# aim-uofa/GenPercept

Measured on AMD Instinct MI355X. Metric: images/sec at 768x768 bf16 (depth), higher is better.
Workload: dtype bf16

## Files before the change

genpercept_amd/csrc/attention.hip:

```cpp
#include <cstdlib>

#include "common.h"
#include "kernels.h"

GP_DEV int attn_off128(int row, int slot) { return row * 128 + ((slot ^ ((row >> 1) & 7)) << 4); }

#ifndef GP_FLASH_DEFER
#define GP_FLASH_DEFER 0.f
#endif
template <int NKB, int NST>
__global__ __launch_bounds__(256, 2) void flash_attn64_kernel(const h16_t* __restrict__ Q, const h16_t* __restrict__ K,
                                                            const h16_t* __restrict__ Vt, h16_t* __restrict__ O, int T, int heads, int ldq,
                                                            int ldk, int Tpad, int ldo) {
    constexpr int KEYS = 32 * NKB, KBYTES = KEYS * 128, NH = NKB / 2;
    constexpr int STAGE = 2 * KBYTES;
    extern __shared__ __attribute__((aligned(16))) char smem[];
    const int tid = threadIdx.x, lane = tid & 63;
    const int wave = __builtin_amdgcn_readfirstlane(tid >> 6);
    const int nqb = (T + 127) >> 7;
    const int sid = xcd_remap(blockIdx.x, gridDim.x);
    const int qb = sid % nqb, bh = sid / nqb;
    const int h = bh % heads, b = bh / heads;
    const int q0 = qb * 128 + wave * 32;
    const int l31 = lane & 31, hh = lane >> 5;
// ... 449 lines not shown
                fr[ks % F5_RD] = lds_frag(sb + (ka0 ^ ((ks & 7) << 5)), (ks >> 3) * 256);
                if ((ks & 3) == 3) ql[(ks >> 2) & 1] = lds_frag(q_lds, (ks >> 2) * 1024);
            };
#pragma unroll
            for (int ks = 0; ks < F5_RD; ++ks) rd(ks);
#pragma unroll
            for (int ks = 0; ks < 32; ++ks) {
                const h16x8_t qv = (ks & 3) != 3 ? qf[3 * (ks >> 2) + ((ks & 3) != 3 ? (ks & 3) : 0)] : ql[(ks >> 2) & 1];
                if (ks & 1) s1 = mfma_32x32x16(fr[ks % F5_RD], qv, ks == 1 ? zero16 : s1);
                else s0 = mfma_32x32x16(fr[ks % F5_RD], qv, ks == 0 ? zero16 : s0);
                if (ks + F5_RD < 32) rd(ks + F5_RD);
                if (do_stage && (ks & 1)) stage_piece(slot_next, kt + 1, ks >> 1);
            }
            f32x16_t s_acc;
#pragma unroll
            for (int r = 0; r < 16; ++r) s_acc[r] = s0[r] + s1[r];
            if (MASK) {
                const int kbase = kt * 32 + 8 * hh;
#pragma unroll
                for (int r = 0; r < 16; ++r)
                    if (kbase + (r & 7) + 16 * (r >> 3) >= T) s_acc[r] = -1e30f;
            }
            float mx = s_acc[0];
#pragma unroll
            for (int r = 1; r < 16; ++r) mx = fmaxf(mx, s_acc[r]);
            mx = fmaxf(mx, other_half(mx));
            const bool moved = __builtin_amdgcn_ballot_w64((mx - m_run) * sc > 8.f) != 0ull;
            if (moved) {
                const float m_new = fmaxf(m_run, mx);
                alpha = __builtin_amdgcn_exp2f((m_run - m_new) * sc);
                m_run = m_new;
                l_run *= alpha;
            }
            const float nm = -m_run * sc;
            float rs = 0.f;
#pragma unroll
            for (int r = 0; r < 16; ++r) {
                s_acc[r] = __builtin_amdgcn_exp2f(__builtin_fmaf(s_acc[r], sc, nm));
                rs += s_acc[r];
            }
            l_run += rs;
#pragma unroll
            for (int j = 0; j < 2; ++j) {
                union { h16x8_t v; unsigned u[4]; } t;
#pragma unroll
                for (int e = 0; e < 4; ++e) t.u[e] = pack_h16x2_ns(s_acc[8 * j + 2 * e], s_acc[8 * j + 2 * e + 1]);
                pf[j] = t.v;
            }
            return moved;
        };
        auto pv_phase = [&](unsigned sb) __attribute__((always_inline)) {
            h16x8_t fr[F5_RD];
            auto rd = [&](int st) __attribute__((always_inline)) { fr[st % F5_RD] = lds_frag(sb + va[st >> 4], (st & 15) * 2048); };
#pragma unroll
            for (int st = 0; st < F5_RD; ++st) rd(st);
#pragma unroll
            for (int st = 0; st < 32; ++st) {
                o_acc[st & 15] = mfma_32x32x16(fr[st % F5_RD], pf[st >> 4], o_acc[st & 15]);
                if (st + F5_RD < 32) rd(st + F5_RD);
            }
        };

        if (t0 < t1) stage(0, t0);
        __builtin_amdgcn_s_waitcnt(0x0070);
        int kt = t0;
        for (;;) {
            bool pending = false;
            unsigned sb = 0;
            for (; kt < t1; ++kt) {
                const int rel = (kt - t0) & 1;
                sb = smem_base + rel * F5_KBYTES;
                wait_vm<0>();
                __builtin_amdgcn_s_barrier();
                const bool nx = kt + 1 < t1;
                const bool moved = (kt * 32 + 32 > T) ? s_phase(sb, kt, nx, rel ^ 1, IC<1>{}) : s_phase(sb, kt, nx, rel ^ 1, IC<0>{});
                if (moved) { pending = true; break; }
                pv_phase(sb);
            }
            if (!pending) break;
#pragma unroll
            for (int d = 0; d < 16; ++d) {
#pragma unroll
                for (int r = 0; r < 16; ++r) o_acc[d][r] *= alpha;
                __builtin_amdgcn_sched_barrier(0);
            }
            pv_phase(sb);
            ++kt;
            __builtin_amdgcn_s_waitcnt(0x0070);
        }
        l_run += other_half(l_run);
        const int q = q0 + l31;
        if (whole) {
            const float inv = 1.f / l_run;
            if (q < T) {
                h16_t* ob = O + ((long long)b * T + q) * ldo;
#pragma unroll
                for (int d = 0; d < 16; ++d)
#pragma unroll
                    for (int g = 0; g < 4; ++g) {
                        const uint2 pk = pack_h16x4(o_acc[d][4 * g] * inv, o_acc[d][4 * g + 1] * inv, o_acc[d][4 * g + 2] * inv, o_acc[d][4 * g + 3] * inv);
                        *(uint2*)(ob + d * 32 + 8 * g + 4 * hh) = pk;
                    }
            }
        } else {
            const long long slot = (long long)(sid / S) * S + part;
            float* po = part_o + (slot * 128 + wave * 32 + l31) * 512;
#pragma unroll
            for (int d = 0; d < 16; ++d)
#pragma unroll
                for (int g = 0; g < 4; ++g)
                    *(float4*)(po + d * 32 + 8 * g + 4 * hh) = float4{o_acc[d][4 * g], o_acc[d][4 * g + 1], o_acc[d][4 * g + 2], o_acc[d][4 * g + 3]};
            if (hh == 0) {
                float* pm = part_ml + (slot * 128 + wave * 32 + l31) * 2;
                pm[0] = m_run;
                pm[1] = l_run;
            }
        }
    }
}

__global__ __launch_bounds__(256) void flash512_combine_kernel(const float* __restrict__ part_o, const float* __restrict__ part_ml,
                                                                h16_t* __restrict__ O, int T, int nqb, int first_blk, int Li, int S, int ldo,
                                                                float scale) {
    const int lb = blockIdx.x >> 2, qq = (blockIdx.x & 3) * 32 + (threadIdx.x >> 3);
    const int b = Li ? lb / Li : (first_blk + lb) / nqb;
    const int q = (Li ? nqb - Li + (lb - b * Li) : first_blk + lb - b * nqb) * 128 + qq;
    if (q >= T) return;
    const float sc = scale * 1.44269504088896340736f;
    float m = -1e30f;
    for (int p = 0; p < S; ++p) m = fmaxf(m, part_ml[(((long long)lb * S + p) * 128 + qq) * 2]);
    float l = 0.f;
    float acc[64];
#pragma unroll
    for (int i = 0; i < 64; ++i) acc[i] = 0.f;
    const int c0 = (threadIdx.x & 7) * 4;
    for (int p = 0; p < S; ++p) {
        const long long row = ((long long)lb * S + p) * 128 + qq;
        const float w = __builtin_amdgcn_exp2f((part_ml[row * 2] - m) * sc);
        l += w * part_ml[row * 2 + 1];
        const float* po = part_o + row * 512 + c0;
#pragma unroll
        for (int i = 0; i < 16; ++i) {
            const float4 v = *(const float4*)(po + 32 * i);
            acc[4 * i] += w * v.x; acc[4 * i + 1] += w * v.y; acc[4 * i + 2] += w * v.z; acc[4 * i + 3] += w * v.w;
        }
    }
    const float inv = 1.f / l;
    h16_t* ob = O + ((long long)b * T + q) * ldo + c0;
#pragma unroll
    for (int i = 0; i < 16; ++i)
        *(uint2*)(ob + 32 * i) = pack_h16x4(acc[4 * i] * inv, acc[4 * i + 1] * inv, acc[4 * i + 2] * inv, acc[4 * i + 3] * inv);
}

bool flash_attn512_supported(int C) { return C == 512 && !gp_sw().no_flash512; }
static int flash512_grid(int nblocks, int ncu, int T) {
    if (nblocks >= ncu) return ncu;
    const int nt = (T + 31) / 32;
    int parts = ncu / nblocks;
    if (parts > nt / 8) parts = nt / 8;
    return parts >= 2 ? parts * nblocks : nblocks;
}
long long flash_attn512_workspace_floats(int B, int T, int ncu) {
    const int nblocks = B * ((T + 127) / 128), G = flash512_grid(nblocks, ncu, T);
    const int L = nblocks % G;
    return L ? (long long)(G / L) * L * 128 * (512 + 2) : 0;
}
void launch_flash_attn512(const h16_t* q, const h16_t* k, const h16_t* vt, h16_t* out, float* ws, int B, int T, int ldq,
                          int ldk, int Tpad, int ldo, float scale, int ncu, hipStream_t s) {
    static unsigned long long attr_mask = 0;
    gp_once_per_device(&attr_mask, [&] { (void)hipFuncSetAttribute((const void*)flash_attn512_kernel, hipFuncAttributeMaxDynamicSharedMemorySize, F5_LDS); });
    const int nqb = (T + 127) / 128, nblocks = B * nqb, G = flash512_grid(nblocks, ncu, T);
    const int rounds = nblocks / G, L = nblocks - rounds * G, S = L ? G / L : 0;
    float* part_o = ws;
    float* part_ml = ws ? ws + (long long)S * L * 128 * 512 : nullptr;
    const int dbg = gp_sw().f5_dbg;
    hipLaunchKernelGGL(flash_attn512_kernel, dim3(G), dim3(256), F5_LDS, s, q, k, vt, out, part_o, part_ml, B, T, ldq, ldk, Tpad,
                       ldo, scale, dbg);
    if (L) hipLaunchKernelGGL(flash512_combine_kernel, dim3(L * 4), dim3(256), 0, s, part_o, part_ml, out, T, nqb, rounds * G, (L % B == 0) ? L / B : 0,
                              S, ldo, scale);
}

__global__ __launch_bounds__(256) void cross_attn_small_kernel(const h16_t* __restrict__ q, const float* __restrict__ kc,
                                                                const float* __restrict__ vc, h16_t* __restrict__ out, long long nrh,
                                                                int C, int heads, int L) {
    const long long idx = (long long)blockIdx.x * 256 + threadIdx.x;
    if (idx >= nrh) return;
    const long long row = idx / heads;
    const int h = (int)(idx - row * heads);
    float qv[64];
    const h16_t* qp = q + row * C + h * 64;
#pragma unroll
    for (int i = 0; i < 8; ++i) {
        const uint4 raw = *(const uint4*)(qp + i * 8);
        const unsigned w[4] = {raw.x, raw.y, raw.z, raw.w};
#pragma unroll
        for (int k = 0; k < 4; ++k) { qv[i * 8 + 2 * k] = h16_lo(w[k]); qv[i * 8 + 2 * k + 1] = h16_hi(w[k]); }
    }
    float o[64];
#pragma unroll
    for (int d = 0; d < 64; ++d) o[d] = 0.f;
    float m = -1e30f, l = 0.f;
    for (int j = 0; j < L; ++j) {
        const float* kp = kc + (long long)j * C + h * 64;
        float s = 0.f;
#pragma unroll
        for (int d = 0; d < 64; ++d) s += qv[d] * kp[d];
        s *= 0.125f;
        const float mn = fmaxf(m, s);
        const float a = __expf(m - mn), pj = __expf(s - mn);
        m = mn;
        l = l * a + pj;
        const float* vp = vc + (long long)j * C + h * 64;
#pragma unroll
        for (int d = 0; d < 64; ++d) o[d] = o[d] * a + pj * vp[d];
    }
    const float inv = 1.f / l;
    h16_t* op = out + row * C + h * 64;
#pragma unroll
    for (int i = 0; i < 8; ++i) {
        uint4 r;
        r.x = pack_h16x2(o[i * 8] * inv, o[i * 8 + 1] * inv);
        r.y = pack_h16x2(o[i * 8 + 2] * inv, o[i * 8 + 3] * inv);
        r.z = pack_h16x2(o[i * 8 + 4] * inv, o[i * 8 + 5] * inv);
        r.w = pack_h16x2(o[i * 8 + 6] * inv, o[i * 8 + 7] * inv);
        *(uint4*)(op + i * 8) = r;
    }
}

void launch_cross_attn_small(const h16_t* q, const float* kc, const float* vc, h16_t* out, int rows, int C, int L, hipStream_t s) {
    const int heads = C / 64;
    const long long nrh = (long long)rows * heads;
    hipLaunchKernelGGL(cross_attn_small_kernel, dim3((unsigned)((nrh + 255) / 256)), dim3(256), 0, s, q, kc, vc, out, nrh, C, heads, L);
}

__global__ __launch_bounds__(256) void softmax_rows_kernel(const float* __restrict__ in, h16_t* __restrict__ out, int T, int ld, float scale) {
    __shared__ float red[8];
    const long long row = blockIdx.x;
    const float* x = in + row * ld;
    h16_t* y = out + row * ld;
    const int tid = threadIdx.x, lane = tid & 63, wv = tid >> 6;
    const float sc = scale * 1.44269504088896340736f;
    float mx = -1e30f;
    for (int i = tid; i < T; i += 256) mx = fmaxf(mx, x[i] * sc);
#pragma unroll
    for (int o = 32; o > 0; o >>= 1) mx = fmaxf(mx, __shfl_xor(mx, o));
    if (lane == 0) red[wv] = mx;
    __syncthreads();
    mx = fmaxf(fmaxf(red[0], red[1]), fmaxf(red[2], red[3]));
    float sum = 0.f;
    for (int i = tid; i < T; i += 256) sum += exp2f(x[i] * sc - mx);
#pragma unroll
    for (int o = 32; o > 0; o >>= 1) sum += __shfl_xor(sum, o);
    if (lane == 0) red[4 + wv] = sum;
    __syncthreads();
    const float inv = 1.f / (red[4] + red[5] + red[6] + red[7]);
    for (int i = tid; i < ld; i += 256) y[i] = i < T ? f_to_h16(exp2f(x[i] * sc - mx) * inv) : (h16_t)0;
}

GP_DEV float4 load4(const float* p, int i) { return ((const float4*)p)[i]; }
GP_DEV float4 load4(const _Float16* p, int i) {
    typedef _Float16 h4_t __attribute__((ext_vector_type(4)));
    const h4_t h = ((const h4_t*)p)[i];
    return make_float4((float)h[0], (float)h[1], (float)h[2], (float)h[3]);
}
template <int NV, typename TIN>
__global__ __launch_bounds__(256) void softmax_rows_reg_kernel(const TIN* __restrict__ in, h16_t* __restrict__ out, int T, int ld, float scale) {
    __shared__ float red[8];
    const long long row = blockIdx.x;
    const TIN* x = in + row * ld;
    uint2* y = (uint2*)(out + row * ld);
    const int tid = threadIdx.x, lane = tid & 63, wv = tid >> 6;
    const float sc = scale * 1.44269504088896340736f;
    const int nvec = ld >> 2;
    float4 v[NV];
    float mx = -1e30f;
#pragma unroll
    for (int k = 0; k < NV; ++k) {
        const int i = k * 256 + tid;
        v[k] = i < nvec ? load4(x, i) : make_float4(0.f, 0.f, 0.f, 0.f);
        const int e0 = i * 4;
        v[k].x = e0 + 0 < T ? v[k].x : -1e30f;
        v[k].y = e0 + 1 < T ? v[k].y : -1e30f;
        v[k].z = e0 + 2 < T ? v[k].z : -1e30f;
        v[k].w = e0 + 3 < T ? v[k].w : -1e30f;
        mx = fmaxf(mx, fmaxf(fmaxf(v[k].x, v[k].y), fmaxf(v[k].z, v[k].w)));
    }
#pragma unroll
    for (int o = 32; o > 0; o >>= 1) mx = fmaxf(mx, __shfl_xor(mx, o));
    if (lane == 0) red[wv] = mx;
    __syncthreads();
    mx = fmaxf(fmaxf(red[0], red[1]), fmaxf(red[2], red[3]));
    const float nm = -mx * sc;
    float sum = 0.f;
#pragma unroll
    for (int k = 0; k < NV; ++k) {
        v[k].x = __builtin_amdgcn_exp2f(__builtin_fmaf(v[k].x, sc, nm));
        v[k].y = __builtin_amdgcn_exp2f(__builtin_fmaf(v[k].y, sc, nm));
        v[k].z = __builtin_amdgcn_exp2f(__builtin_fmaf(v[k].z, sc, nm));
        v[k].w = __builtin_amdgcn_exp2f(__builtin_fmaf(v[k].w, sc, nm));
        sum += (v[k].x + v[k].y) + (v[k].z + v[k].w);
    }
#pragma unroll
    for (int o = 32; o > 0; o >>= 1) sum += __shfl_xor(sum, o);
    if (lane == 0) red[4 + wv] = sum;
    __syncthreads();
    const float inv = 1.f / (red[4] + red[5] + red[6] + red[7]);
#pragma unroll
    for (int k = 0; k < NV; ++k) {
        const int i = k * 256 + tid;
        if (i < nvec) y[i] = pack_h16x4(v[k].x * inv, v[k].y * inv, v[k].z * inv, v[k].w * inv);
    }
}

void launch_softmax_rows(const float* in, h16_t* out, int rows, int T, int ld, float scale, hipStream_t s) {
    if ((ld & 3) == 0 && scale > 0.f && ld <= 16384) {
        if (ld <= 4096) hipLaunchKernelGGL((softmax_rows_reg_kernel<4, float>), dim3(rows), dim3(256), 0, s, in, out, T, ld, scale);
        else if (ld <= 9216) hipLaunchKernelGGL((softmax_rows_reg_kernel<9, float>), dim3(rows), dim3(256), 0, s, in, out, T, ld, scale);
        else hipLaunchKernelGGL((softmax_rows_reg_kernel<16, float>), dim3(rows), dim3(256), 0, s, in, out, T, ld, scale);
        return;
    }
    hipLaunchKernelGGL(softmax_rows_kernel, dim3(rows), dim3(256), 0, s, in, out, T, ld, scale);
}

bool softmax_rows_f16_supported(int ld) { return (ld & 3) == 0 && ld <= 16384; }
void launch_softmax_rows_f16(const void* in, h16_t* out, int rows, int T, int ld, float scale, hipStream_t s) {
    const _Float16* x = (const _Float16*)in;
    if (ld <= 4096) hipLaunchKernelGGL((softmax_rows_reg_kernel<4, _Float16>), dim3(rows), dim3(256), 0, s, x, out, T, ld, scale);
    else if (ld <= 9216) hipLaunchKernelGGL((softmax_rows_reg_kernel<9, _Float16>), dim3(rows), dim3(256), 0, s, x, out, T, ld, scale);
    else hipLaunchKernelGGL((softmax_rows_reg_kernel<16, _Float16>), dim3(rows), dim3(256), 0, s, x, out, T, ld, scale);
}
// ... 3 lines not shown
```

genpercept_amd/csrc/igemm.hip:

```cpp
#include <cstdlib>
#include <cstring>

#include "common.h"
#include "epilogue.h"
#include "kernels.h"

#include <atomic>

std::mutex& gp_attr_mutex() {
    static std::mutex m;
    return m;
}

static GpSwitches g_switches = [] {
    GpSwitches s{};
    s.gn_fuse_max_slices = s.gn_fuse_below_px = s.vt_tile = s.xfold_lds = -1;
    s.qkv_fuse_max_rows = 1 << 30;
    return s;
}();
const GpSwitches& gp_sw() { return g_switches; }
void gp_switches_reload() {
    auto flag = [](const char* n) { return getenv(n) != nullptr ? 1 : 0; };
    auto num = [](const char* n, int dflt) { const char* v = getenv(n); return v ? atoi(v) : dflt; };
    GpSwitches s{};
    s.flash_ring3 = flag("GENPERCEPT_FLASH_RING3");
    s.no_flash512 = flag("GENPERCEPT_NO_FLASH512");
    s.f5_dbg = num("GENPERCEPT_F5_DBG", 0);
    s.no_conv_few = flag("GENPERCEPT_NO_CONV_FEW");
    s.no_conv_img = flag("GENPERCEPT_NO_CONV_IMG");
    s.conv_img_s = num("GENPERCEPT_CONV_IMG_S", 0);
    s.no_cross_fold = flag("GENPERCEPT_NO_CROSS_FOLD");
    s.no_gn_fusion = flag("GENPERCEPT_NO_GN_FUSION");
    s.gn_fuse_max_slices = num("GENPERCEPT_GN_FUSE_MAX_SLICES", -1);
    s.gn_fuse_below_px = num("GENPERCEPT_GN_FUSE_BELOW_PX", -1);
    s.no_stats_fusion = flag("GENPERCEPT_NO_STATS_FUSION");
    s.vt_tile = num("GENPERCEPT_VT_TILE", -1);
    s.no_gn_small = flag("GENPERCEPT_NO_GN_SMALL");
    s.fp32_scores = flag("GENPERCEPT_FP32_SCORES");
    s.no_qkv_fuse = flag("GENPERCEPT_NO_QKV_FUSE");
    s.qkv_fuse_max_rows = num("GENPERCEPT_QKV_FUSE_MAX_ROWS", 1 << 30);
    s.no_rgb_conv = flag("GENPERCEPT_NO_RGB_CONV");
    s.igemm_dbg = num("GENPERCEPT_IGEMM_DBG", 0);
    s.no_splitk = flag("GENPERCEPT_NO_SPLITK");
    s.no_halo = flag("GENPERCEPT_NO_HALO");
    s.no_pgemm = flag("GENPERCEPT_NO_PGEMM");
    s.gn_apply_old = flag("GENPERCEPT_GN_APPLY_OLD");
    s.no_up_phases = flag("GENPERCEPT_NO_UP_PHASES");
    s.gn_small_old = flag("GENPERCEPT_GN_SMALL_OLD");
    s.xfold_lds = num("GENPERCEPT_XFOLD_LDS", -1);
    s.no_fin_fuse = flag("GENPERCEPT_NO_FIN_FUSE");
    s.c_no_flash = flag("GENPERCEPT_C_NO_FLASH");
    s.pgemm_ring3 = flag("GENPERCEPT_PGEMM_RING3");
    static std::mutex mu;
    std::lock_guard<std::mutex> lk(mu);
    if (memcmp(&g_switches, &s, sizeof(s)) != 0) g_switches = s;
}

constexpr bool PRIO = true;
template <int N>
GP_DEV void wait_vm_n() { asm volatile("s_waitcnt vmcnt(%0)" ::"n"(N) : "memory"); }

template <int BM, int BN, int WM, int WN, int KS, int NSTAGE>
__global__ __launch_bounds__(64 * WM * WN) void igemm_kernel(const IGemmParams p) {
    constexpr int NW = WM * WN;
    constexpr int TM = BM / WM, TN = BN / WN;
    constexpr int FM = TM / 16, FN = TN / 16, FP = FN / 2;
    constexpr int A_IT = BM / (8 * NW), B_IT = BN / (8 * NW);
    constexpr int LPS = A_IT + B_IT;
    constexpr int A_BYTES = BM * 128, STAGE = (BM + BN) * 128;
    constexpr bool CONV = KS != 1, UPS = KS == 4;
    static_assert((NW == 4 || NW == 8) && TM % 16 == 0 && TN % 32 == 0 && BM % (8 * NW) == 0 && BN % (8 * NW) == 0, "tile shape");
    static_assert(NSTAGE >= 2 && NSTAGE <= 4, "ring depth");
    extern __shared__ __attribute__((aligned(16))) char smem[];

    const int tid = threadIdx.x, lane = tid & 63;
    const int wave = __builtin_amdgcn_readfirstlane(tid >> 6);
    const int wm = wave / WN, wn = wave % WN;
    const bool second_half = wave >= NW / 2;

    const int ncols = p.N > p.n_store ? p.N : p.n_store;
    const int tiles_n = (ncols + BN - 1) / BN, tiles_m = (p.M + BM - 1) / BM;
    const int sid = xcd_remap(blockIdx.x, tiles_m * tiles_n);
    const int m0 = (sid / tiles_n) * BM, n0 = (sid % tiles_n) * BN;
    const int z = blockIdx.y;

    const h16_t* in = p.in + (long long)z * p.in_bs;
    const h16_t* wt = p.wt + (long long)z * p.wt_bs;
    const int Cin = p.Cin;
    const int cpt = Cin >> 6;
    const int nk_all = (CONV ? 9 : 1) * cpt;
    const int zs = p.ksplit > 1 ? (int)blockIdx.z : 0;
    const int k_begin = p.ksplit > 1 ? (int)((long long)nk_all * zs / p.ksplit) : 0;
    const int nk = p.ksplit > 1 ? (int)((long long)nk_all * (zs + 1) / p.ksplit) - k_begin : nk_all;

    const int chunk_a = (lane & 7) ^ (lane >> 3);
    const int chunk_w = (lane & 7) ^ (((lane >> 4) & 1) | ((wave & 1) << 1) | (((wave >> 1) & 1) << 2));
    const h16_t* zsrc_a = p.zero + chunk_a * 8;
    const h16_t* zsrc_w = p.zero + chunk_w * 8;

    const h16_t* a_base[A_IT];
    unsigned a_mask[A_IT];
    int a_y0[UPS ? A_IT : 1], a_x0[UPS ? A_IT : 1];
    const h16_t* a_tap[UPS ? A_IT : 1];
#pragma unroll
    for (int i = 0; i < A_IT; ++i) {
        const int m = m0 + (wave + NW * i) * 8 + (lane >> 3);
        const bool ok = m < p.M;
        if (!CONV) {
            a_base[i] = in + (long long)m * p.lda + chunk_a * 8;
            a_mask[i] = ok ? 1u : 0u;
        } else {
            const int hw = p.Ho * p.Wo;
            const int b = m / hw, rem = m - b * hw;
            const int oy = rem / p.Wo, ox = rem - oy * p.Wo;
            const int y0 = oy * p.stride - p.pad_t, x0 = ox * p.stride - p.pad_l;
            const h16_t* img = in + (long long)b * p.Hi * p.Wi * Cin + chunk_a * 8;
            unsigned mk = 0;
            const int hlim = UPS ? p.Hu : p.Hi, wlim = UPS ? p.Wu : p.Wi;
#pragma unroll
            for (int t = 0; t < 9; ++t)
                if (ok && (unsigned)(y0 + t / 3) < (unsigned)hlim && (unsigned)(x0 + t % 3) < (unsigned)wlim) mk |= 1u << t;
            a_mask[i] = mk;
            if constexpr (UPS) {
                a_base[i] = img;
                a_y0[i] = y0;
                a_x0[i] = x0;
                a_tap[i] = img;
            } else {
                a_base[i] = img + ((long long)y0 * p.Wi + x0) * Cin;
            }
        }
    }
    const h16_t* w_base[B_IT];
    bool w_ok[B_IT];
#pragma unroll
    for (int i = 0; i < B_IT; ++i) {
        const int n = n0 + (wave + NW * i) * 8 + (lane >> 3);
        w_ok[i] = n < p.n_rows;
        w_base[i] = wt + (long long)n * p.ldw + chunk_w * 8;
    }
    const float ups_sy = UPS ? (float)p.Hi / (float)p.Hu : 1.f;
    const float ups_sx = UPS ? (float)p.Wi / (float)p.Wu : 1.f;

    int st_tap = CONV ? k_begin / cpt : 0, st_cc = CONV ? k_begin - st_tap * cpt : k_begin;
    int st_ky = st_tap / 3, st_kx = st_tap - 3 * st_ky;
    auto stage = [&](int buf) {
        char* sb = smem + buf * STAGE;
        if constexpr (UPS) {
          if (st_cc == 0) {
#pragma unroll
            for (int i = 0; i < A_IT; ++i) {
                const int iy = min((int)floorf((float)(a_y0[i] + st_ky) * ups_sy), p.Hi - 1);
                const int ix = min((int)floorf((float)(a_x0[i] + st_kx) * ups_sx), p.Wi - 1);
                a_tap[i] = a_base[i] + ((long long)iy * p.Wi + ix) * Cin;
            }
          }
        }
        const int koff = st_cc << 6;
        const long long aoff = CONV && !UPS ? (long long)(st_ky * p.Wi + st_kx) * Cin + koff : koff;
#pragma unroll
        for (int i = 0; i < A_IT; ++i) {
            const bool ok = (a_mask[i] >> st_tap) & 1u;
            const h16_t* ab;
            if constexpr (UPS) ab = a_tap[i]; else ab = a_base[i];
            const h16_t* src = ok ? ab + aoff : zsrc_a;
            glds16(src, sb + (wave + NW * i) * 1024);
        }
        const int woff = st_tap * Cin + koff;
#pragma unroll
        for (int i = 0; i < B_IT; ++i) {
            const h16_t* src = w_ok[i] ? w_base[i] + woff : zsrc_w;
            glds16(src, sb + A_BYTES + (wave + NW * i) * 1024);
        }
        if (++st_cc == cpt) {
            st_cc = 0;
            if (CONV) {
                ++st_tap;
                if (++st_kx == 3) { st_kx = 0; ++st_ky; }
            }
        }
// ... 245 lines not shown
```

genpercept_amd/csrc/kernels.h:

```cpp
#pragma once
#include <hip/hip_runtime.h>
#include <stdint.h>

#include <mutex>

#ifndef GP_F16
#define GP_F16 0
#endif
typedef unsigned short h16_t;

enum { GP_ACT_NONE = 0, GP_ACT_SILU = 1, GP_ACT_RELU = 2, GP_ACT_GEGLU = 3 };
enum { GP_BIAS_NONE = 0, GP_BIAS_COL = 1, GP_BIAS_ROW = 2 };

struct IGemmParams {
    const h16_t* in;
    const h16_t* wt;
    const float* bias;
    const h16_t* res;
    void* out;
    const h16_t* zero;
    const float* in_scale;
    const float* in_shift;
    int in_silu;
    float* stats_out;
    int M, N, Cin;
    int n_rows;
    int ks;
    int B, Hi, Wi, Ho, Wo;
    int stride, pad_t, pad_l;
    int ups;
    int Hu, Wu;
    int lda, ldo, ldres;
    int ldw;
    int n_store;
    int out_fp32;
    int act, bias_mode;
    int dbg;
    float* splitk_ws;
    long long splitk_ws_floats;
    int batch;
    int ksplit;
    long long split_bs;
    long long in_bs, wt_bs, out_bs, res_bs, bias_bs;
    h16_t* vt_out;
    int vt_col0, vt_T, vt_Tpad;
    const h16_t* wt_ph;
    int res_f32;
};

struct GpSwitches {
    int flash_ring3, no_flash512, f5_dbg, no_conv_few, no_conv_img, conv_img_s, no_cross_fold, no_gn_fusion, gn_fuse_max_slices,
        gn_fuse_below_px, no_stats_fusion, vt_tile, no_gn_small, fp32_scores, no_qkv_fuse, qkv_fuse_max_rows, no_rgb_conv, igemm_dbg, no_splitk,
        no_halo, no_pgemm, gn_apply_old, xfold_lds, no_fin_fuse, pgemm_ring3, gn_small_old, no_up_phases, c_no_flash;
};
const GpSwitches& gp_sw();
void gp_switches_reload();

void* gp_sat_flag_addr_igemm();
void* gp_sat_flag_addr_conv_halo();
void* gp_sat_flag_addr_pgemm();
void* gp_sat_flag_addr_conv_few();
void* gp_sat_flag_addr_norm();
void* gp_sat_flag_addr_attention();
void* gp_sat_flag_addr_elementwise();
#define GP_SAT_TUS {gp_sat_flag_addr_igemm, gp_sat_flag_addr_conv_halo, gp_sat_flag_addr_pgemm, gp_sat_flag_addr_conv_few, gp_sat_flag_addr_norm, gp_sat_flag_addr_attention, gp_sat_flag_addr_elementwise}

void launch_igemm(const IGemmParams& p, int tile_hint, hipStream_t s);
int igemm_ksplit(const IGemmParams& p, int tile_hint);
std::mutex& gp_attr_mutex();
template <typename F>
inline void gp_once_per_device(unsigned long long* mask, F&& f) {
    int dev = 0;
    if (hipGetDevice(&dev) != hipSuccess || dev < 0 || dev > 63) { f(); return; }
    const unsigned long long bit = 1ull << dev;
    if (__atomic_load_n(mask, __ATOMIC_ACQUIRE) & bit) return;
    std::lock_guard<std::mutex> lk(gp_attr_mutex());
    if (__atomic_load_n(mask, __ATOMIC_RELAXED) & bit) return;
    f();
    __atomic_store_n(mask, __atomic_load_n(mask, __ATOMIC_RELAXED) | bit, __ATOMIC_RELEASE);
}
bool pgemm_applicable(const IGemmParams& p);
int pgemm_bm(const IGemmParams& p);
void launch_pgemm(const IGemmParams& p, hipStream_t s);
bool igemm_uses_pgemm(const IGemmParams& p, int tile_hint);
bool conv_halo_applicable(const IGemmParams& p);
void launch_conv_halo(const IGemmParams& p, hipStream_t s);
bool conv_uses_halo(const IGemmParams& p, int tile_hint);
bool conv_halo_uses_phases(const IGemmParams& p);
int conv_halo_stat_rows(const IGemmParams& p);
int igemm_tile_info(const IGemmParams& p, int tile_hint, int* mode, int* bm);
void launch_groupnorm_from_partials(const float* partials, int mode, int bm, int B, int H, int W, int C, int G, float eps, const float* gamma,
                                    const float* beta, float* scale, float* shift, hipStream_t s);

void launch_groupnorm_stats(const h16_t* x, const float* gamma, const float* beta, int B, int HW, int C, int G, float eps, float* ws,
                            float* scale, float* shift, hipStream_t s);
void launch_groupnorm_apply(const h16_t* x, h16_t* y, const float* scale, const float* shift, int B, int HW, int C, int silu, hipStream_t s);
void launch_groupnorm(const h16_t* x, h16_t* y, const float* gamma, const float* beta, int B, int HW, int C, int G, float eps,
                      int silu, float* ws, hipStream_t s);
int groupnorm_ws_floats(int B, int HW, int C, int G);
bool groupnorm_small_applicable(int B, int HW, int C, int G);
void launch_groupnorm_small(const h16_t* x, h16_t* y, const float* gamma, const float* beta, int B, int HW, int C, int G, float eps, int silu,
                            hipStream_t s);

void launch_layernorm(const h16_t* x, h16_t* y, const float* gamma, const float* beta, int rows, int C, float eps, hipStream_t s);

void launch_flash_attn64(const h16_t* q, const h16_t* k, const h16_t* vt, h16_t* out, int B, int T, int heads,
                         int ldq, int ldk, int Tpad, int ldo, hipStream_t s);
bool flash_attn512_supported(int C);
long long flash_attn512_workspace_floats(int B, int T, int ncu);
void launch_flash_attn512(const h16_t* q, const h16_t* k, const h16_t* vt, h16_t* out, float* ws, int B, int T, int ldq,
                          int ldk, int Tpad, int ldo, float scale, int ncu, hipStream_t s);

void launch_cross_attn_small(const h16_t* q, const float* kc, const float* vc, h16_t* out, int rows, int C, int L, hipStream_t s);

bool cross_attn_fold_supported(int C, int heads);
void launch_cross_attn_fold(const h16_t* y, h16_t* y_out, h16_t* n3_out, const float* U, const float* u0, const float* G, const float* c0,
                            const float* g3, const float* b3, int rows, int C, int heads, float eps, hipStream_t s);

void launch_softmax_rows(const float* in, h16_t* out, int rows, int T, int ld, float scale, hipStream_t s);
bool softmax_rows_f16_supported(int ld);
void launch_softmax_rows_f16(const void* in_f16, h16_t* out, int rows, int T, int ld, float scale, hipStream_t s);

void launch_rgb_prologue(const void* rgb, int is_u8, h16_t* out, int B, int H, int W, int Cpad, hipStream_t s);
int rgb_conv_in_rows(int B, int H, int W);
void launch_pack_k27(const h16_t* wt, int ldw, int Cout, h16_t* w27, hipStream_t s);
void launch_rgb_conv_in(const void* rgb, int is_u8, const h16_t* w27, const float* bias, h16_t* out, float* stats, int B, int H, int W, int Cout,
                        hipStream_t s);
void launch_concat(const h16_t* a, int Ca, const h16_t* b, int Cb, h16_t* out, long long pixels, hipStream_t s);
int concat_stats_bm(long long hw, long long pixels, int channels);
void launch_concat_stats(const h16_t* a, int Ca, const h16_t* b, int Cb, h16_t* out, long long pixels, int bm, float* part, hipStream_t s);
struct DdimCoef { float x0_sample, x0_model, eps_sample, eps_model, prev_x0, prev_eps, clip; };
void launch_ddim_init(const float* noise_nchw, h16_t* lat, float* sample, int B, int H, int W, int L, int ld, int off, hipStream_t s);
void launch_ddim_step(const h16_t* model, int ldm, float* sample, h16_t* uin, int ldu, int off, h16_t* x0_out, int ldx, long long pixels, int L,
                      const DdimCoef& k, hipStream_t s);
void launch_nchw_f32_to_nhwc(const float* in, h16_t* out, int B, int C, int H, int W, int Cpad, hipStream_t s);
void launch_nhwc_to_nchw_f32(const h16_t* in, float* out, int B, int C, int H, int W, int ld, hipStream_t s);
void launch_decode_epilogue(const h16_t* in, float* out, int B, int H, int W, int ld, int mean3, int raw, hipStream_t s);
void launch_scale_pad(const h16_t* in, h16_t* out, long long pixels, int C, int ldi, int ldo, float scale, hipStream_t s);
void launch_pointwise_small(const h16_t* in, h16_t* out, const float* w, const float* bias, long long pixels, int Cin, int Cout, int ldi,
                            int ldo, float in_scale, hipStream_t s);
void launch_relu(const h16_t* in, h16_t* out, long long n, hipStream_t s);
void launch_add(const h16_t* a, const h16_t* b, h16_t* out, long long n, hipStream_t s);
void launch_bilinear(const h16_t* in, h16_t* out, int B, int Hi, int Wi, int Ho, int Wo, int C, int align_corners, hipStream_t s);
void launch_dpt_final(const h16_t* in, const float* w, float bias, float* out, int B, int HW, int Cin, hipStream_t s);
void launch_minmax_norm(float* x, int B, long long n, float* ws, hipStream_t s);

bool conv_img_applicable(const IGemmParams& p);
int conv_img_ksplit(const IGemmParams& p);
void launch_conv_img(const IGemmParams& p, float* part, int S, hipStream_t s);

bool conv_few_applicable(int Cin, int Cout, int H, int W);
void launch_conv_few(const h16_t* in, const h16_t* wt, const float* bias, const float* scale, const float* shift, const h16_t* zero, float* out, int B,
                     int H, int W, int silu, int mean3, int raw, int ncu, hipStream_t s);

void launch_resize(const void* in, void* out, float* tmp, long long planes, int Hi, int Wi, int Ho, int Wo, int mode, int u8, int clip01, hipStream_t s);
void launch_clip01(const float* in, float* out, long long n, hipStream_t s);
void launch_normalize_rgb(const float* in, float* out, long long n, hipStream_t s);
void launch_colorize_lut(const float* x, const unsigned char* lut, unsigned char* rgb, long long n, hipStream_t s);
void launch_quantize(const float* x, void* q, long long n, int bits, hipStream_t s);

void launch_c_split3(const float* x, int ldx, h16_t* out, long long rows, int C, int b_order, int act, float scale, hipStream_t s);
void launch_c_rgb_split(const void* rgb, int is_u8, h16_t* out, int B, int H, int W, hipStream_t s);
int c_gn_stat_rows(int HW, int C, int* bm_out);
void launch_c_gn_stats(const float* x, float* part, int B, int HW, int C, hipStream_t s);
void launch_c_gn_apply_split(const float* x, h16_t* out, const float* scale, const float* shift, int B, int HW, int C, int silu, hipStream_t s);
void launch_c_layernorm_split(const float* x, h16_t* out, const float* gamma, const float* beta, int rows, int C, float eps, hipStream_t s);
void launch_c_concat(const float* a, int Ca, const float* b, int Cb, float* out, long long pixels, hipStream_t s);
void launch_c_heads_split(const float* qkv, int ld, h16_t* Qs, h16_t* Ks, h16_t* Vts, int B, int T, int Tpad, int heads, int hd, hipStream_t s);
void launch_c_qkv_planes(const float* qkv, int ld, h16_t* qk_hi, h16_t* qk_lo, h16_t* vt_hi, h16_t* vt_lo, int B, int T, int Tpad, int heads, int hd,
                         hipStream_t s);
void launch_flash_attn64_split(const h16_t* qk_hi, const h16_t* qk_lo, const h16_t* vt_hi, const h16_t* vt_lo, h16_t* out, int B, int T, int heads, int ld,
                               int Tpad, hipStream_t s);
bool c_softmax_split_supported(int ld);
void launch_c_softmax_split(const float* in, h16_t* out, long long rows, int T, int ld, float scale, hipStream_t s);
void launch_c_heads_merge_split(const float* O, h16_t* out, int B, int T, int heads, int hd, hipStream_t s);
bool c_cross_fold_supported(int C);
void launch_c_cross_fold(const float* y, float* y_out, h16_t* n3_out, const float* U, const float* u0, const float* G, const float* c0, const float* g3,
                         const float* b3, int rows, int C, int heads, float eps, hipStream_t s);
void launch_c_cross_attn_small(const float* q, const float* kc, const float* vc, h16_t* out, int rows, int C, int L, hipStream_t s);
void launch_c_pointwise_small(const float* in, float* out, const float* w, const float* bias, long long pixels, int Cin, int Cout, int ldi, int ldo,
                              float in_scale, hipStream_t s);
void launch_c_decode_epilogue(const float* in, float* out, int B, int H, int W, int ld, int mean3, int raw, hipStream_t s);
void launch_c_nchw_to_nhwc(const float* in, float* out, int B, int C, int H, int W, int Cpad, hipStream_t s);
void launch_c_nhwc_to_nchw(const float* in, float* out, int B, int C, int H, int W, int ld, hipStream_t s);
void launch_c_add(const float* a, const float* b, float* out, long long n, hipStream_t s);
void launch_c_bilinear(const float* in, float* out, int B, int Hi, int Wi, int Ho, int Wo, int C, int align_corners, hipStream_t s);
void launch_c_dpt_final(const float* in, const float* w, float bias, float* out, int B, int HW, int Cin, hipStream_t s);
void launch_c_ddim_init(const float* noise_nchw, float* lat, float* sample, int B, int H, int W, int L, int ld, int off, hipStream_t s);
void launch_c_ddim_step(const float* model, int ldm, float* sample, float* uin, int ldu, int off, float* x0_out, int ldx, long long pixels, int L,
                        const DdimCoef& k, hipStream_t s);

double mfma_peak_tflops(int ms_target, hipStream_t s, int shape = 0);
double mfma_lds_probe_tflops(int reads_per_16_mfma, int waves_per_simd, int mode, hipStream_t s);
```

Measured before the change: 93.14.

## Add 8-wave split-head-dim flash attention kernel for C=512

Adds a new 512-thread flash attention kernel for the single-head 512-dim attention. Each pair of waves splits the head dimension in half and exchanges partial QK scores through LDS before the softmax, so each wave keeps half as many accumulators and more waves per block can overlap work. It also skips the output rescale when the running max moves by less than a threshold, and raises the priority of one wave group. This kernel becomes the default, replacing the 256-thread kernel, which remains reachable through an env switch. The extra cost is a cross-wave score exchange and barrier on every key tile.

```diff
diff --git a/genpercept_amd/csrc/attention.hip b/genpercept_amd/csrc/attention.hip
--- a/genpercept_amd/csrc/attention.hip
+++ b/genpercept_amd/csrc/attention.hip
@@ -625,6 +625,258 @@
         *(uint2*)(ob + 32 * i) = pack_h16x4(acc[4 * i] * inv, acc[4 * i + 1] * inv, acc[4 * i + 2] * inv, acc[4 * i + 3] * inv);
 }
 
+constexpr int F8_XBYTES = 4096;
+constexpr int F8_LDS = 4 * F5_KBYTES + 8 * F8_XBYTES;
+
+GP_DEV unsigned opaque(unsigned x) { asm volatile("" : "+v"(x)); return x; }
+
+template <bool PRIO, bool ST>
+__global__ __launch_bounds__(512) void flash_attn512x8_kernel(const h16_t* __restrict__ Q, const h16_t* __restrict__ K,
+                                                               const h16_t* __restrict__ Vt, h16_t* __restrict__ O,
+                                                               float* __restrict__ part_o, float* __restrict__ part_ml, int B, int T,
+                                                               int ldq, int ldk, int Tpad, int ldo, float scale) {
+    extern __shared__ __attribute__((aligned(16))) char smem[];
+    const int tid = threadIdx.x, lane = tid & 63;
+    const int wave = __builtin_amdgcn_readfirstlane(tid >> 6);
+    const int pr = ST ? wave >> 1 : wave & 3, hf = ST ? wave & 1 : wave >> 2, grp = wave >> 2;
+    const int l31 = lane & 31, hh = lane >> 5;
+    const int nqb = (T + 127) >> 7, nblocks = B * nqb, G = gridDim.x;
+    const int nt = (T + 31) >> 5;
+    const int rounds = nblocks / G, L = nblocks - rounds * G, S = L ? G / L : 0;
+    const int sid = xcd_remap(blockIdx.x, G);
+    const unsigned smem_base = (unsigned)(unsigned long long)smem;
+    const float sc = scale * 1.44269504088896340736f;
+    f32x16_t zero16;
+#pragma unroll
+    for (int r = 0; r < 16; ++r) zero16[r] = 0.f;
+    if (PRIO && grp) __builtin_amdgcn_s_setprio(1);
+    const unsigned xw = smem_base + 4 * F5_KBYTES + wave * F8_XBYTES + lane * 16;
+    const unsigned xr = smem_base + 4 * F5_KBYTES + (ST ? wave ^ 1 : wave ^ 4) * F8_XBYTES + lane * 16;
+
+    const int items = rounds + ((L && sid / S < L) ? 1 : 0);
+    for (int it = 0; it < items; ++it) {
+        const bool whole = it < rounds;
+        const int part = whole ? 0 : sid % S;
+        const int t0 = whole ? 0 : (int)((long long)nt * part / S), t1 = whole ? nt : (int)((long long)nt * (part + 1) / S);
+        const int Li = (L % B == 0) ? L / B : 0;
+        int b, qb;
+        if (whole) {
+            const int w = it * G + sid, per = nqb - Li;
+            b = Li ? w / per : w / nqb;
+            qb = Li ? w - b * per : w - b * nqb;
+        } else {
+            const int lb = sid / S;
+            b = Li ? lb / Li : (rounds * G + lb) / nqb;
+            qb = Li ? nqb - Li + (lb - b * Li) : rounds * G + lb - b * nqb;
+        }
+        const int q0 = qb * 128 + pr * 32;
+        const h16_t* Qb = Q + (long long)b * T * ldq;
+        const h16_t* Kb = K + (long long)b * T * ldk;
+        const h16_t* Vb = Vt + (long long)b * 512 * Tpad;
+
+        __syncthreads();
+        h16x8_t qf[16];
+        {
+            const int q = q0 + l31;
+            const bool ok = q < T;
+#pragma unroll
+            for (int j = 0; j < 16; ++j) {
+                qf[j] = h16x8_t{0, 0, 0, 0, 0, 0, 0, 0};
+                if (ok) qf[j] = *(const h16x8_t*)(Qb + (long long)q * ldq + hf * 256 + j * 16 + hh * 8);
+            }
+            asm volatile("" ::"v"(qf[15]));
+        }
+        const buf_rsrc_t k_rs = make_rsrc(Kb, (unsigned)((long long)T * ldk * 2));
+        const buf_rsrc_t v_rs = make_rsrc(Vb, (unsigned)(512ll * Tpad * 2));
+        const unsigned k_lane = (unsigned)lane << 4;
+        const unsigned v_lane_off = ((unsigned)(lane >> 2) * Tpad + (((lane & 3) ^ ((lane >> 4) & 3)) << 3)) * 2;
+        auto stage_piece = [&](int slot, int kt, int pc) __attribute__((always_inline)) {
+            char* sb = smem + slot * F5_KBYTES;
+            if (pc < 4) {
+                const int i = wave * 4 + pc;
+                const int key = min(kt * 32 + pi23(i), T - 1);
+                blds16(k_rs, opaque(k_lane) ^ ((unsigned)(i & 15) << 4), (unsigned)key * (unsigned)(ldk * 2), sb + i * 1024);
+            } else {
+                const int m = pc - 4;
+                blds16(v_rs, opaque(v_lane_off), (unsigned)((64 * wave + 16 * m) * Tpad + kt * 32) * 2u, sb + 2 * F5_KBYTES + (wave * 4 + m) * 1024);
+            }
+        };
+        auto stage = [&](int slot, int kt) __attribute__((always_inline)) {
+#pragma unroll
+            for (int pc = 0; pc < 8; ++pc) stage_piece(slot, kt, pc);
+        };
+
+        f32x16_t o_acc[8];
+#pragma unroll
+        for (int d = 0; d < 8; ++d) o_acc[d] = zero16;
+        float m_run = -1e30f, l_run = 0.f, alpha = 1.f;
+        const unsigned ka0 = l31 * 1024 + ((hh ^ (l31 & 15)) << 4);
+        unsigned va[2];
+#pragma unroll
+        for (int j = 0; j < 2; ++j) va[j] = 2 * F5_KBYTES + hf * 8 * 2048 + l31 * 64 + (((2 * j + hh) ^ ((l31 >> 2) & 3)) << 4);
+        h16x8_t pf[2];
+        constexpr int NP = ST ? 4 : 8;
+        constexpr int F8_RD = ST ? 2 : 4;
+        auto stage_in = [&](int j, int st_kt, int st_pc0) __attribute__((always_inline)) {
+            if (st_kt >= 0 && (j % (16 / NP)) == 16 / NP - 1) stage_piece((st_kt - t0) & 1, st_kt, st_pc0 + j / (16 / NP));
+        };
+        auto s_phase = [&](unsigned sb, int kt, int st_kt, int st_pc0, auto maskc) __attribute__((always_inline)) -> bool {
+            constexpr bool MASK = decltype(maskc)::value != 0;
+            const unsigned kb = sb + hf * 512, ka = opaque(ka0);
+            f32x16_t s_acc;
+            h16x8_t fr[F8_RD];
+            auto rd = [&](int j) __attribute__((always_inline)) { fr[j % F8_RD] = lds_frag(kb + (ka ^ ((j & 7) << 5)), (j >> 3) * 256); };
+#pragma unroll
+            for (int j = 0; j < F8_RD; ++j) rd(j);
+#pragma unroll
+            for (int j = 0; j < 16; ++j) {
+                s_acc = mfma_32x32x16(fr[j % F8_RD], qf[j], j == 0 ? zero16 : s_acc);
+                if (j + F8_RD < 16) rd(j + F8_RD);
+                stage_in(j, st_kt, st_pc0);
+            }
+#pragma unroll
+            for (int g = 0; g < 4; ++g) *(lds_f4_ptr)(opaque(xw) + g * 1024) = f32x4_t{s_acc[4 * g], s_acc[4 * g + 1], s_acc[4 * g + 2], s_acc[4 * g + 3]};
+            if (ST && st_kt >= 0) wait_vm<4>();
+            else if (ST) wait_vm<0>();
+            asm volatile("s_waitcnt lgkmcnt(0)\n\ts_barrier" ::: "memory");
+#pragma unroll
+            for (int g = 0; g < 4; ++g) {
+                const f32x4_t o = *(lds_f4_ptr)(opaque(xr) + g * 1024);
+#pragma unroll
+                for (int e = 0; e < 4; ++e) s_acc[4 * g + e] += o[e];
+            }
+            if (MASK) {
+                const int kbase = kt * 32 + 8 * hh;
+#pragma unroll
+                for (int r = 0; r < 16; ++r)
+                    if (kbase + (r & 7) + 16 * (r >> 3) >= T) s_acc[r] = -1e30f;
+            }
+            float mx = s_acc[0];
+#pragma unroll
+            for (int r = 1; r < 16; ++r) mx = fmaxf(mx, s_acc[r]);
+            mx = fmaxf(mx, other_half(mx));
+            const bool moved = __builtin_amdgcn_ballot_w64((mx - m_run) * sc > 8.f) != 0ull;
+            if (moved) {
+                const float m_new = fmaxf(m_run, mx);
+                alpha = __builtin_amdgcn_exp2f((m_run - m_new) * sc);
+                m_run = m_new;
+                l_run *= alpha;
+            }
+            const float nm = -m_run * sc;
+            float rs = 0.f;
+#pragma unroll
+            for (int r = 0; r < 16; ++r) {
+                s_acc[r] = __builtin_amdgcn_exp2f(__builtin_fmaf(s_acc[r], sc, nm));
+                rs += s_acc[r];
+            }
+            l_run += rs;
+#pragma unroll
+            for (int j = 0; j < 2; ++j) {
+                union { h16x8_t v; unsigned u[4]; } t;
+#pragma unroll
+                for (int e = 0; e < 4; ++e) t.u[e] = pack_h16x2_ns(s_acc[8 * j + 2 * e], s_acc[8 * j + 2 * e + 1]);
+                pf[j] = t.v;
+            }
+            return moved;
+        };
+        auto pv_phase = [&](unsigned sb, int st_kt, int st_pc0) __attribute__((always_inline)) {
+            h16x8_t fr[F8_RD];
+            auto rd = [&](int st) __attribute__((always_inline)) { fr[st % F8_RD] = lds_frag(sb + va[st >> 3], (st & 7) * 2048); };
+#pragma unroll
+            for (int st = 0; st < F8_RD; ++st) rd(st);
+#pragma unroll
+            for (int st = 0; st < 16; ++st) {
+                o_acc[st & 7] = mfma_32x32x16(fr[st % F8_RD], pf[st >> 3], o_acc[st & 7]);
+                if (st + F8_RD < 16) rd(st + F8_RD);
+                if (ST) stage_in(st, st_kt, st_pc0);
+            }
+        };
+
+        if (t0 < t1) stage(0, t0);
+        bool iss = t0 < t1;
+        auto sync = [&]() __attribute__((always_inline)) {
+            if (iss) wait_vm<4>(); else wait_vm<0>();
+            asm volatile("s_waitcnt lgkmcnt(0)\n\ts_barrier" ::: "memory");
+            iss = false;
+        };
+        if (ST && grp) {
+            sync();
+            if (t0 + 1 < t1) {
+#pragma unroll
+                for (int pc = 0; pc < 4; ++pc) stage_piece(1, t0 + 1, pc);
+                iss = true;
+            }
+        }
+        __builtin_amdgcn_s_waitcnt(0x0070);
+        int kt = t0;
+        for (;;) {
+            bool pending = false;
+            unsigned sb = 0;
+            int pv_kt = -1, pv_pc0 = 0;
+            for (; kt < t1; ++kt) {
+                const int rel = (kt - t0) & 1;
+                sb = smem_base + rel * F5_KBYTES;
+                if (ST) {
+                    sync();
+                } else {
+                    wait_vm<0>();
+                    __builtin_amdgcn_s_barrier();
+                }
+                const int s_kt = kt + 1 < t1 ? kt + 1 : -1, s_pc0 = ST && grp ? 4 : 0;
+                if (ST) {
+                    pv_kt = grp ? (kt + 2 < t1 ? kt + 2 : -1) : s_kt;
+                    pv_pc0 = grp ? 0 : 4;
+                }
+                const bool moved = (kt * 32 + 32 > T) ? s_phase(sb, kt, s_kt, s_pc0, IC<1>{}) : s_phase(sb, kt, s_kt, s_pc0, IC<0>{});
+                if (ST) iss = false;
+                if (moved) { pending = true; break; }
+                pv_phase(sb, pv_kt, pv_pc0);
+                if (ST) iss = pv_kt >= 0;
+            }
+            if (!pending) break;
+#pragma unroll
+            for (int d = 0; d < 8; ++d) {
+#pragma unroll
+                for (int r = 0; r < 16; ++r) o_acc[d][r] *= alpha;
+                __builtin_amdgcn_sched_barrier(0);
+            }
+            pv_phase(sb, pv_kt, pv_pc0);
+            if (ST) iss = pv_kt >= 0;
+            ++kt;
+            __builtin_amdgcn_s_waitcnt(0x0070);
+        }
+        if (ST && !grp) sync();
+        l_run += other_half(l_run);
+        const int q = q0 + l31;
+        if (whole) {
+            const float inv = 1.f / l_run;
+            if (q < T) {
+                h16_t* ob = O + ((long long)b * T + q) * ldo + hf * 256;
+#pragma unroll
+                for (int d = 0; d < 8; ++d)
+#pragma unroll
+                    for (int g = 0; g < 4; ++g) {
+                        const uint2 pk = pack_h16x4(o_acc[d][4 * g] * inv, o_acc[d][4 * g + 1] * inv, o_acc[d][4 * g + 2] * inv, o_acc[d][4 * g + 3] * inv);
+                        *(uint2*)(ob + d * 32 + 8 * g + 4 * hh) = pk;
+                    }
+            }
+        } else {
+            const long long slot = (long long)(sid / S) * S + part;
+            float* po = part_o + (slot * 128 + pr * 32 + l31) * 512 + hf * 256;
+#pragma unroll
+            for (int d = 0; d < 8; ++d)
+#pragma unroll
+                for (int g = 0; g < 4; ++g)
+                    *(float4*)(po + d * 32 + 8 * g + 4 * hh) = float4{o_acc[d][4 * g], o_acc[d][4 * g + 1], o_acc[d][4 * g + 2], o_acc[d][4 * g + 3]};
+            if (hf == 0 && hh == 0) {
+                float* pm = part_ml + (slot * 128 + pr * 32 + l31) * 2;
+                pm[0] = m_run;
+                pm[1] = l_run;
+            }
+        }
+    }
+}
+
 bool flash_attn512_supported(int C) { return C == 512 && !gp_sw().no_flash512; }
 static int flash512_grid(int nblocks, int ncu, int T) {
     if (nblocks >= ncu) return ncu;
@@ -641,14 +893,31 @@
 void launch_flash_attn512(const h16_t* q, const h16_t* k, const h16_t* vt, h16_t* out, float* ws, int B, int T, int ldq,
                           int ldk, int Tpad, int ldo, float scale, int ncu, hipStream_t s) {
     static unsigned long long attr_mask = 0;
-    gp_once_per_device(&attr_mask, [&] { (void)hipFuncSetAttribute((const void*)flash_attn512_kernel, hipFuncAttributeMaxDynamicSharedMemorySize, F5_LDS); });
+    gp_once_per_device(&attr_mask, [&] {
+        (void)hipFuncSetAttribute((const void*)flash_attn512_kernel, hipFuncAttributeMaxDynamicSharedMemorySize, F5_LDS);
+        (void)hipFuncSetAttribute((const void*)flash_attn512x8_kernel<true, true>, hipFuncAttributeMaxDynamicSharedMemorySize, F8_LDS);
+        (void)hipFuncSetAttribute((const void*)flash_attn512x8_kernel<false, false>, hipFuncAttributeMaxDynamicSharedMemorySize, F8_LDS);
+        (void)hipFuncSetAttribute((const void*)flash_attn512x8_kernel<true, false>, hipFuncAttributeMaxDynamicSharedMemorySize, F8_LDS);
+    });
     const int nqb = (T + 127) / 128, nblocks = B * nqb, G = flash512_grid(nblocks, ncu, T);
     const int rounds = nblocks / G, L = nblocks - rounds * G, S = L ? G / L : 0;
     float* part_o = ws;
     float* part_ml = ws ? ws + (long long)S * L * 128 * 512 : nullptr;
-    const int dbg = gp_sw().f5_dbg;
-    hipLaunchKernelGGL(flash_attn512_kernel, dim3(G), dim3(256), F5_LDS, s, q, k, vt, out, part_o, part_ml, B, T, ldq, ldk, Tpad,
-                       ldo, scale, dbg);
+    const GpSwitches& sw = gp_sw();
+    if (sw.flash512_v1) {
+        const int dbg = sw.f5_dbg;
+        hipLaunchKernelGGL(flash_attn512_kernel, dim3(G), dim3(256), F5_LDS, s, q, k, vt, out, part_o, part_ml, B, T, ldq, ldk, Tpad,
+                           ldo, scale, dbg);
+    } else if (sw.f8_stagger) {
+        hipLaunchKernelGGL((flash_attn512x8_kernel<true, true>), dim3(G), dim3(512), F8_LDS, s, q, k, vt, out, part_o, part_ml, B, T, ldq,
+                           ldk, Tpad, ldo, scale);
+    } else if (sw.f8_noprio) {
+        hipLaunchKernelGGL((flash_attn512x8_kernel<false, false>), dim3(G), dim3(512), F8_LDS, s, q, k, vt, out, part_o, part_ml, B, T, ldq,
+                           ldk, Tpad, ldo, scale);
+    } else {
+        hipLaunchKernelGGL((flash_attn512x8_kernel<true, false>), dim3(G), dim3(512), F8_LDS, s, q, k, vt, out, part_o, part_ml, B, T, ldq,
+                           ldk, Tpad, ldo, scale);
+    }
     if (L) hipLaunchKernelGGL(flash512_combine_kernel, dim3(L * 4), dim3(256), 0, s, part_o, part_ml, out, T, nqb, rounds * G, (L % B == 0) ? L / B : 0,
                               S, ldo, scale);
 }
diff --git a/genpercept_amd/csrc/igemm.hip b/genpercept_amd/csrc/igemm.hip
--- a/genpercept_amd/csrc/igemm.hip
+++ b/genpercept_amd/csrc/igemm.hip
@@ -26,6 +26,9 @@
     s.flash_ring3 = flag("GENPERCEPT_FLASH_RING3");
     s.no_flash512 = flag("GENPERCEPT_NO_FLASH512");
     s.f5_dbg = num("GENPERCEPT_F5_DBG", 0);
+    s.flash512_v1 = flag("GENPERCEPT_FLASH512_V1");
+    s.f8_noprio = flag("GENPERCEPT_F8_NOPRIO");
+    s.f8_stagger = flag("GENPERCEPT_F8_STAGGER");
     s.no_conv_few = flag("GENPERCEPT_NO_CONV_FEW");
     s.no_conv_img = flag("GENPERCEPT_NO_CONV_IMG");
     s.conv_img_s = num("GENPERCEPT_CONV_IMG_S", 0);
diff --git a/genpercept_amd/csrc/kernels.h b/genpercept_amd/csrc/kernels.h
--- a/genpercept_amd/csrc/kernels.h
+++ b/genpercept_amd/csrc/kernels.h
@@ -51,7 +51,8 @@
 struct GpSwitches {
     int flash_ring3, no_flash512, f5_dbg, no_conv_few, no_conv_img, conv_img_s, no_cross_fold, no_gn_fusion, gn_fuse_max_slices,
         gn_fuse_below_px, no_stats_fusion, vt_tile, no_gn_small, fp32_scores, no_qkv_fuse, qkv_fuse_max_rows, no_rgb_conv, igemm_dbg, no_splitk,
-        no_halo, no_pgemm, gn_apply_old, xfold_lds, no_fin_fuse, pgemm_ring3, gn_small_old, no_up_phases, c_no_flash;
+        no_halo, no_pgemm, gn_apply_old, xfold_lds, no_fin_fuse, pgemm_ring3, gn_small_old, no_up_phases, c_no_flash,
+        flash512_v1, f8_noprio, f8_stagger;
 };
 const GpSwitches& gp_sw();
 void gp_switches_reload();
```

After: 93.84 (median of 6 runs). No clear change (+0.8%).
